# CGuerreroCordova/HydroDEM

Measured on AMD Instinct MI355X. Metric: Mcells/s sink-fill+D8 on 16384^2 float32 DEM, higher is better.
Workload: dtype f32; 1 GPU; 16384x16384 float32 synthetic DEM (SURVEY 8d 'rough': plane + 4 sinusoids + 0.5 m noise + 0.1% pits), SinkFill eps=0 to exact convergence + D8; 16384 rows per GPU, row-block partition; rows_per_gpu=16384, cols=16384, tiles=70225, visits_unchanged=25634, visits_flat=2843, certifying_rounds=0, halo_exchanges=0

## Files before the change

### hydrodem_amd/csrc/hdem_stencil.hip

```cpp
#include "hdem_internal.h"

namespace {

constexpr int TW = 256;
constexpr int TH = 32;
template <typename T> struct tile_rows { static constexpr int value = sizeof(T) == 8 ? TH / 2 : TH; };
constexpr int LS = TW + 8;
constexpr int NT = 256;

__device__ __forceinline__ int reflect(int i, int n)
{
    while (i < 0 || i >= n) {
        if (i < 0) i = -i - 1;
        if (i >= n) i = 2 * n - 1 - i;
    }
    return i;
}

template <typename T, bool REFLECT>
__device__ __forceinline__ void stage_tile(const T *__restrict__ src, int H, int W,
                                           int y0, int x0, T *t)
{
    constexpr int THT = tile_rows<T>::value;
    constexpr int V = 16 / sizeof(T);
    constexpr int CPR = TW / V;
    typedef T vec_t __attribute__((ext_vector_type(V)));
    typedef T vecu_t __attribute__((ext_vector_type(V), aligned(sizeof(T))));
    const int tid = threadIdx.x;
    constexpr int CHUNKS = ((THT + 2) * CPR + NT - 1) / NT;
    vec_t v[CHUNKS];
#pragma unroll
    for (int j = 0; j < CHUNKS; ++j) {
        const int i = tid + j * NT;
        const int r = i / CPR, c = (i % CPR) * V;
        int gy = y0 - 1 + r;
        const int gx = x0 + c;
        const bool row_ok = gy >= 0 && gy < H;
        if (REFLECT) gy = reflect(gy, H);
        if (i >= (THT + 2) * CPR) {
            v[j] = vec_t(T(0));
        } else if ((row_ok || REFLECT) && gx + V <= W) {
            v[j] = *reinterpret_cast<const vecu_t *>(src + (size_t)gy * W + gx);
        } else {
            for (int k = 0; k < V; ++k) {
                int xx = gx + k;
                T e = T(0);
                if (REFLECT) e = src[(size_t)gy * W + reflect(xx, W)];
                else if (row_ok && xx < W) e = src[(size_t)gy * W + xx];
                v[j][k] = e;
            }
        }
    }
#pragma unroll
    for (int j = 0; j < CHUNKS; ++j) {
        const int i = tid + j * NT;
        if (i < (THT + 2) * CPR)
            *reinterpret_cast<vec_t *>(t + (i / CPR) * LS + 4 + (i % CPR) * V) = v[j];
    }
    for (int i = tid; i < (THT + 2) * 2; i += NT) {
        int r = i >> 1, side = i & 1;
        int gy = y0 - 1 + r, gx = side ? x0 + TW : x0 - 1;
        T e = T(0);
        if (REFLECT) e = src[(size_t)reflect(gy, H) * W + reflect(gx, W)];
        else if (gy >= 0 && gy < H && gx >= 0 && gx < W) e = src[(size_t)gy * W + gx];
        t[r * LS + (side ? 4 + TW : 3)] = e;
    }
}

template <typename T>
__device__ __forceinline__ void read_row6(const T *t, int r, int cg, T (&o)[6])
{
    const T *p = t + r * LS + 4 + 4 * cg;
    o[0] = p[-1];
    o[1] = p[0]; o[2] = p[1]; o[3] = p[2]; o[4] = p[3];
    o[5] = p[4];
}

__device__ __forceinline__ unsigned d8_code(float nw, float n, float ne, float w,
                                            float c, float e, float sw, float s,
                                            float se)
{
    const float dg = 0.70710678f;
    float best = 0.0f;
    unsigned code = 0;
    float d;
    d = (c - nw) * dg; if (d > best) { best = d; code = 32; }
    d = (c - n);       if (d > best) { best = d; code = 64; }
    d = (c - ne) * dg; if (d > best) { best = d; code = 128; }
    d = (c - w);       if (d > best) { best = d; code = 16; }
    d = (c - e);       if (d > best) { best = d; code = 1; }
    d = (c - sw) * dg; if (d > best) { best = d; code = 8; }
    d = (c - s);       if (d > best) { best = d; code = 4; }
    d = (c - se) * dg; if (d > best) { best = d; code = 2; }
    return code;
}

__global__ __launch_bounds__(NT) void d8_kernel(const float *__restrict__ z, int H,
                                               int W, uint8_t *__restrict__ out,
                                               int tiles_x, int vec_store)
{
    __shared__ __attribute__((aligned(16))) float t[(TH + 2) * LS];
    const int bx = blockIdx.x % tiles_x, by = blockIdx.x / tiles_x;
    const int x0 = bx * TW, y0 = by * TH;
    stage_tile<float, false>(z, H, W, y0, x0, t);
    __syncthreads();

    const int cg = threadIdx.x & 63, rg = threadIdx.x >> 6;
    const int x = x0 + 4 * cg;
    if (x >= W) return;
    float a[6], b[6], c[6];
    read_row6(t, rg * 8 + 0, cg, a);
    read_row6(t, rg * 8 + 1, cg, b);
#pragma unroll
    for (int rr = 0; rr < 8; ++rr) {
        const int y = y0 + rg * 8 + rr;
        read_row6(t, rg * 8 + rr + 2, cg, c);
        if (y < H) {
            unsigned code[4];
#pragma unroll
            for (int k = 0; k < 4; ++k) {
                unsigned cd = d8_code(a[k], a[k + 1], a[k + 2], b[k], b[k + 1],
                                      b[k + 2], c[k], c[k + 1], c[k + 2]);
                int xx = x + k;
                bool interior = y > 0 && y < H - 1 && xx > 0 && xx < W - 1;
                code[k] = interior ? cd : 0u;
            }
            uint8_t *o = out + (size_t)y * W + x;
            if (vec_store && x + 4 <= W) {
                *reinterpret_cast<uint32_t *>(o) =
                    code[0] | (code[1] << 8) | (code[2] << 16) | (code[3] << 24);
            } else {
#pragma unroll
                for (int k = 0; k < 4; ++k)
                    if (x + k < W) o[k] = (uint8_t)code[k];
            }
        }
#pragma unroll
        for (int k = 0; k < 6; ++k) { a[k] = b[k]; b[k] = c[k]; }
    }
}

template <bool HAS_EPS>
__global__ __launch_bounds__(NT) void certify_d8_kernel(const float *__restrict__ z,
                                                       const float *__restrict__ w, int H, int W,
                                                       float eps, uint8_t *__restrict__ out,
                                                       int tiles_x, int vec_store, int *flag)
{
    __shared__ __attribute__((aligned(16))) float t[(TH + 2) * LS];
    const int bx = blockIdx.x % tiles_x, by = blockIdx.x / tiles_x;
    const int x0 = bx * TW, y0 = by * TH;
    stage_tile<float, false>(w, H, W, y0, x0, t);
    __syncthreads();

    const int cg = threadIdx.x & 63, rg = threadIdx.x >> 6;
    const int x = x0 + 4 * cg;
    if (x >= W) return;
    float zc[8][4];
#pragma unroll
    for (int rr = 0; rr < 8; ++rr) {
        const int y = min(y0 + rg * 8 + rr, H - 1);
        if (x + 4 <= W) {
            const hdem_f4 m = hdem_ld4u(z + (size_t)y * W + x);
            zc[rr][0] = m[0]; zc[rr][1] = m[1]; zc[rr][2] = m[2]; zc[rr][3] = m[3];
        } else {
#pragma unroll
            for (int k = 0; k < 4; ++k) zc[rr][k] = z[(size_t)y * W + min(x + k, W - 1)];
        }
    }
    bool lower = false;
    float a[6], b[6], c[6];
    read_row6(t, rg * 8 + 0, cg, a);
    read_row6(t, rg * 8 + 1, cg, b);
#pragma unroll
    for (int rr = 0; rr < 8; ++rr) {
        const int y = y0 + rg * 8 + rr;
        read_row6(t, rg * 8 + rr + 2, cg, c);
        if (y < H) {
            unsigned code[4];
#pragma unroll
            for (int k = 0; k < 4; ++k) {
                const int xx = x + k;
                const bool interior = y > 0 && y < H - 1 && xx > 0 && xx < W - 1;
                float m = fminf(fminf(fminf(a[k], a[k + 1]), fminf(a[k + 2], b[k])),
                                fminf(fminf(b[k + 1], b[k + 2]), fminf(c[k], fminf(c[k + 1], c[k + 2]))));
                m = fminf(m, HDEM_INF);
                if (HAS_EPS) m += eps;
                const float wc = fminf(b[k + 1], HDEM_INF), zz = fminf(zc[rr][k], HDEM_INF);
                lower |= interior && __builtin_amdgcn_fmed3f(zz, wc, m) != wc;
                const unsigned cd = d8_code(a[k], a[k + 1], a[k + 2], b[k], b[k + 1], b[k + 2], c[k],
                                            c[k + 1], c[k + 2]);
                code[k] = interior ? cd : 0u;
            }
            if (out) {
                uint8_t *o = out + (size_t)y * W + x;
                if (vec_store && x + 4 <= W) {
                    *reinterpret_cast<uint32_t *>(o) =
                        code[0] | (code[1] << 8) | (code[2] << 16) | (code[3] << 24);
                } else {
#pragma unroll
                    for (int k = 0; k < 4; ++k)
                        if (x + k < W) o[k] = (uint8_t)code[k];
                }
            }
        }
#pragma unroll
        for (int k = 0; k < 6; ++k) { a[k] = b[k]; b[k] = c[k]; }
    }
    if (lower) *flag = 1;
}

template <typename T>
__device__ __forceinline__ T mean9(const T (&a)[6], const T (&b)[6], const T (&c)[6],
                                   int k, int do_round)
{
    double acc = 0.0;
    acc += (double)a[k]; acc += (double)a[k + 1]; acc += (double)a[k + 2];
    acc += (double)b[k]; acc += (double)b[k + 1]; acc += (double)b[k + 2];
    acc += (double)c[k]; acc += (double)c[k + 1]; acc += (double)c[k + 2];
    T s = (T)acc;
    T m = s / T(9);
    if (do_round) m = sizeof(T) == 4 ? (T)rintf((float)m) : (T)rint((double)m);
    return m;
}

template <typename T>
__global__ __launch_bounds__(NT) void boxmean3_kernel(const T *__restrict__ x, int H,
                                                     int W, T *__restrict__ out,
                                                     int tiles_x, int do_round)
{
    constexpr int THT = tile_rows<T>::value;
    constexpr int RPW = THT / 4;
    __shared__ __attribute__((aligned(16))) T t[(THT + 2) * LS];
    const int bx = blockIdx.x % tiles_x, by = blockIdx.x / tiles_x;
    const int x0 = bx * TW, y0 = by * THT;
    stage_tile<T, true>(x, H, W, y0, x0, t);
    __syncthreads();

    const int cg = threadIdx.x & 63, rg = threadIdx.x >> 6;
    const int xc = x0 + 4 * cg;
    if (xc >= W) return;
    T a[6], b[6], c[6];
    read_row6(t, rg * RPW + 0, cg, a);
    read_row6(t, rg * RPW + 1, cg, b);
#pragma unroll
    for (int rr = 0; rr < RPW; ++rr) {
        const int y = y0 + rg * RPW + rr;
        read_row6(t, rg * RPW + rr + 2, cg, c);
        if (y < H) {
            T m[4];
#pragma unroll
            for (int k = 0; k < 4; ++k) m[k] = mean9<T>(a, b, c, k, do_round);
            T *o = out + (size_t)y * W + xc;
            if (xc + 4 <= W) {
                if (sizeof(T) == 4) {
                    hdem_f4 v = {(float)m[0], (float)m[1], (float)m[2], (float)m[3]};
                    hdem_st4u(reinterpret_cast<float *>(o), v);
                } else {
                    o[0] = m[0]; o[1] = m[1]; o[2] = m[2]; o[3] = m[3];
                }
            } else {
#pragma unroll
                for (int k = 0; k < 4; ++k)
                    if (xc + k < W) o[k] = m[k];
            }
        }
#pragma unroll
        for (int k = 0; k < 6; ++k) { a[k] = b[k]; b[k] = c[k]; }
    }
}

template <typename T>
__global__ __launch_bounds__(NT) void convolve_kernel(const T *__restrict__ x, int H,
                                                     int W, const double *__restrict__ wt,
                                                     int kh, int kw, T *__restrict__ out)
{
    size_t i = (size_t)blockIdx.x * NT + threadIdx.x;
    if (i >= (size_t)H * W) return;
    int y = (int)(i / W), xx = (int)(i % W);
    int py = kh / 2, px = kw / 2;
    double acc = 0.0;
    for (int j = 0; j < kh; ++j) {
        int gy = reflect(y + j - py, H);
        for (int k = 0; k < kw; ++k) {
            double w = wt[(kh - 1 - j) * kw + (kw - 1 - k)];
            if (w != 0.0)
                acc += (double)x[(size_t)gy * W + reflect(xx + k - px, W)] * w;
        }
    }
    const T s = (T)acc;
    out[i] = s / (T)(kh * kw);
}

template <typename T>
__global__ __launch_bounds__(NT) void around_kernel(const T *x, int64_t n, T *out)
{
    int64_t i = (int64_t)blockIdx.x * NT + threadIdx.x;
    if (i < n) out[i] = sizeof(T) == 4 ? (T)rintf((float)x[i]) : (T)rint((double)x[i]);
}

inline int tiles_of(int H, int W, int th, int *tx)
{
    *tx = (W + TW - 1) / TW;
    return *tx * ((H + th - 1) / th);
}

}

int hdem_certify_d8_launch(hdem_ctx *ctx, const float *z, const float *w, int H, int W, float eps,
                           uint8_t *d8, int *flag)
{
    int tx, nt = tiles_of(H, W, TH, &tx);
    const int vec = d8 && (W % 4 == 0) && ((uintptr_t)d8 % 4 == 0);
    if (eps != 0.0f)
        hipLaunchKernelGGL(certify_d8_kernel<true>, dim3(nt), dim3(NT), 0, ctx->stream, z, w, H, W,
                           eps, d8, tx, vec, flag);
    else
        hipLaunchKernelGGL(certify_d8_kernel<false>, dim3(nt), dim3(NT), 0, ctx->stream, z, w, H, W,
                           eps, d8, tx, vec, flag);
    HDEM_HIP_CHECK(hipGetLastError());
    return HDEM_OK;
}

extern "C" int hdem_d8_f32_dev(hdem_ctx *ctx, const float *z, int H, int W, uint8_t *out)
{
    if (int rc = hdem_check_call(ctx, z, out, H, W)) return rc;
    HDEM_HIP_CHECK(hipSetDevice(ctx->device));
    int tx, nt = tiles_of(H, W, TH, &tx);
    int vec = (W % 4 == 0) && ((uintptr_t)out % 4 == 0);
    {
        hdem_scoped_timer tm(ctx, HDEM_K_D8, (int64_t)H * W);
        hipLaunchKernelGGL(d8_kernel, dim3(nt), dim3(NT), 0, ctx->stream, z, H, W, out,
                           tx, vec);
    }
    HDEM_HIP_CHECK(hipGetLastError());
    return HDEM_OK;
}

extern "C" int hdem_d8_f32(hdem_ctx *ctx, const float *z, int H, int W, uint8_t *out)
{
    if (int rc = hdem_check_call(ctx, z, out, H, W)) return rc;
    HDEM_HIP_CHECK(hipSetDevice(ctx->device));
    size_t n = (size_t)H * W;
    hdem_dbuf dz, dout;
    if (int rc = dz.upload(ctx, z, n * sizeof(float))) return rc;
    if (int rc = dout.alloc(ctx, n)) return rc;
    if (int rc = hdem_d8_f32_dev(ctx, dz.as<const float>(), H, W, dout.as<uint8_t>())) return rc;
    return dout.download(out, n);
}

template <typename T>
static int boxmean_dev(hdem_ctx *ctx, const T *x, int H, int W, int do_round, T *out)
{
    if (int rc = hdem_check_call(ctx, x, out, H, W)) return rc;
    HDEM_REQUIRE((const void *)x != (const void *)out, HDEM_ERR_BAD_ARG,
                 "box mean cannot run in place");
    HDEM_HIP_CHECK(hipSetDevice(ctx->device));
    int tx, nt = tiles_of(H, W, tile_rows<T>::value, &tx);
    {
        hdem_scoped_timer tm(ctx, HDEM_K_BOXMEAN, (int64_t)H * W);
        hipLaunchKernelGGL(boxmean3_kernel<T>, dim3(nt), dim3(NT), 0, ctx->stream, x, H, W,
                           out, tx, do_round);
    }
    HDEM_HIP_CHECK(hipGetLastError());
    return HDEM_OK;
}

template <typename T>
static int boxmean_host(hdem_ctx *ctx, const T *x, int H, int W, int do_round, T *out)
{
    if (int rc = hdem_check_call(ctx, x, out, H, W)) return rc;
    HDEM_HIP_CHECK(hipSetDevice(ctx->device));
    size_t bytes = (size_t)H * W * sizeof(T);
    hdem_dbuf dx, dout;
    if (int rc = dx.upload(ctx, x, bytes)) return rc;
    if (int rc = dout.alloc(ctx, bytes)) return rc;
    if (int rc = boxmean_dev<T>(ctx, dx.as<const T>(), H, W, do_round, dout.as<T>())) return rc;
    return dout.download(out, bytes);
}

extern "C" int hdem_boxmean3_f32_dev(hdem_ctx *c, const float *x, int H, int W, int r, float *o)
{ return boxmean_dev<float>(c, x, H, W, r, o); }
extern "C" int hdem_boxmean3_f64_dev(hdem_ctx *c, const double *x, int H, int W, int r, double *o)
{ return boxmean_dev<double>(c, x, H, W, r, o); }
extern "C" int hdem_boxmean3_f32(hdem_ctx *c, const float *x, int H, int W, int r, float *o)
{ return boxmean_host<float>(c, x, H, W, r, o); }
extern "C" int hdem_boxmean3_f64(hdem_ctx *c, const double *x, int H, int W, int r, double *o)
{ return boxmean_host<double>(c, x, H, W, r, o); }

template <typename T>
static int convolve_host(hdem_ctx *ctx, const T *x, int H, int W, const double *weights, int kh,
                         int kw, T *out)
{
    if (int rc = hdem_check_call(ctx, x, out, H, W)) return rc;
    HDEM_REQUIRE(weights, HDEM_ERR_BAD_ARG, "weights is null");
    HDEM_REQUIRE(kh > 0 && kw > 0 && kh <= 15 && kw <= 15, HDEM_ERR_BAD_ARG,
                 "weights shape %d x %d not supported (1..15 per axis)", kh, kw);
    HDEM_REQUIRE(kh % 2 == 1 && kw % 2 == 1, HDEM_ERR_WINDOW_EVEN,
                 "weights shape %d x %d must be odd on both axes", kh, kw);
    HDEM_HIP_CHECK(hipSetDevice(ctx->device));
    size_t n = (size_t)H * W, bytes = n * sizeof(T);
    hdem_dbuf dx, dout, dw;
    if (int rc = dx.upload(ctx, x, bytes)) return rc;
    if (int rc = dw.upload(ctx, weights, sizeof(double) * kh * kw)) return rc;
    if (int rc = dout.alloc(ctx, bytes)) return rc;
    {
        hdem_scoped_timer tm(ctx, HDEM_K_CONVOLVE, (int64_t)n);
        hipLaunchKernelGGL(convolve_kernel<T>, dim3((unsigned)((n + NT - 1) / NT)), dim3(NT), 0,
                           ctx->stream, dx.as<const T>(), H, W, dw.as<const double>(), kh, kw,
                           dout.as<T>());
    }
    HDEM_HIP_CHECK(hipGetLastError());
    return dout.download(out, bytes);
}

extern "C" int hdem_convolve_f32(hdem_ctx *ctx, const float *x, int H, int W,
                                 const double *weights, int kh, int kw, float *out)
{ return convolve_host<float>(ctx, x, H, W, weights, kh, kw, out); }
extern "C" int hdem_convolve_f64(hdem_ctx *ctx, const double *x, int H, int W,
                                 const double *weights, int kh, int kw, double *out)
{ return convolve_host<double>(ctx, x, H, W, weights, kh, kw, out); }

template <typename T>
static int around_host(hdem_ctx *ctx, const T *x, int64_t n, T *out)
{
    HDEM_REQUIRE(ctx && x && out, HDEM_ERR_BAD_ARG, "null argument");
    HDEM_REQUIRE(n > 0, HDEM_ERR_BAD_ARG, "n must be positive");
    HDEM_HIP_CHECK(hipSetDevice(ctx->device));
    const size_t bytes = (size_t)n * sizeof(T);
    hdem_dbuf dx;
    if (int rc = dx.upload(ctx, x, bytes)) return rc;
    hipLaunchKernelGGL(around_kernel<T>, dim3((unsigned)((n + NT - 1) / NT)), dim3(NT), 0,
                       ctx->stream, dx.as<const T>(), n, dx.as<T>());
    HDEM_HIP_CHECK(hipGetLastError());
    return dx.download(out, bytes);
}

extern "C" int hdem_around_f32(hdem_ctx *c, const float *x, int64_t n, float *o)
{ return around_host<float>(c, x, n, o); }
extern "C" int hdem_around_f64(hdem_ctx *c, const double *x, int64_t n, double *o)
{ return around_host<double>(c, x, n, o); }
```

Baseline: 63880 Mcells/s.

## Share neighbor slope differences across rows and batch D8 stores

Restructures the D8 and certify-D8 kernels so that vertical and diagonal differences between adjacent rows are computed once and reused by the rows above and below. Direction selection becomes a max reduction followed by equality-based code selection. For eps=0 the certify check is reduced to a cheaper comparison built from the drop mask. Codes for all 8 rows are buffered in registers and stored at the end, with sched_barriers to control instruction scheduling. This trims ALU work and branching per cell, at the cost of more registers and a tie-breaking rule that must match the original strict-greater ordering.

After: 63790 Mcells/s. About the same (-0.1%).

```diff
diff --git a/hydrodem_amd/csrc/hdem_stencil.hip b/hydrodem_amd/csrc/hdem_stencil.hip
--- a/hydrodem_amd/csrc/hdem_stencil.hip
+++ b/hydrodem_amd/csrc/hdem_stencil.hip
@@ -76,23 +76,88 @@
     o[5] = p[4];
 }
 
-__device__ __forceinline__ unsigned d8_code(float nw, float n, float ne, float w,
-                                            float c, float e, float sw, float s,
-                                            float se)
+struct d8_link {
+    float v[4];
+    float dr[5];
+    float dl[5];
+};
+
+__device__ __forceinline__ void d8_link_rows(const float (&u)[6], const float (&l)[6],
+                                             d8_link &s)
 {
     const float dg = 0.70710678f;
-    float best = 0.0f;
-    unsigned code = 0;
-    float d;
-    d = (c - nw) * dg; if (d > best) { best = d; code = 32; }
-    d = (c - n);       if (d > best) { best = d; code = 64; }
-    d = (c - ne) * dg; if (d > best) { best = d; code = 128; }
-    d = (c - w);       if (d > best) { best = d; code = 16; }
-    d = (c - e);       if (d > best) { best = d; code = 1; }
-    d = (c - sw) * dg; if (d > best) { best = d; code = 8; }
-    d = (c - s);       if (d > best) { best = d; code = 4; }
-    d = (c - se) * dg; if (d > best) { best = d; code = 2; }
-    return code;
+#pragma unroll
+    for (int k = 0; k < 4; ++k) s.v[k] = u[k + 1] - l[k + 1];
+#pragma unroll
+    for (int j = 0; j < 5; ++j) {
+        s.dr[j] = (u[j] - l[j + 1]) * dg;
+        s.dl[j] = (u[j + 1] - l[j]) * dg;
+    }
+}
+
+__device__ __forceinline__ void d8_row4(const float (&b)[6], const d8_link &n,
+                                        const d8_link &s, unsigned (&code)[4],
+                                        bool (&drop)[4])
+{
+    float h[5];
+#pragma unroll
+    for (int j = 0; j < 5; ++j) h[j] = b[j] - b[j + 1];
+#pragma unroll
+    for (int k = 0; k < 4; ++k) {
+        const float d0 = -n.dr[k], d1 = -n.v[k], d2 = -n.dl[k + 1], d3 = -h[k];
+        const float d4 = h[k + 1], d5 = s.dl[k], d6 = s.v[k], d7 = s.dr[k + 1];
+        float m = __builtin_fmaxf(__builtin_fmaxf(d0, d1), d2);
+        m = __builtin_fmaxf(__builtin_fmaxf(m, d3), d4);
+        m = __builtin_fmaxf(__builtin_fmaxf(m, d5), d6);
+        m = __builtin_fmaxf(m, d7);
+        unsigned cd = d7 == m ? 2u : 0u;
+        cd = d6 == m ? 4u : cd;
+        cd = d5 == m ? 8u : cd;
+        cd = d4 == m ? 1u : cd;
+        cd = d3 == m ? 16u : cd;
+        cd = d2 == m ? 128u : cd;
+        cd = d1 == m ? 64u : cd;
+        cd = d0 == m ? 32u : cd;
+        code[k] = cd;
+        drop[k] = m > 0.0f;
+    }
+}
+
+__device__ __forceinline__ unsigned d8_column_mask(int x, int W)
+{
+    unsigned m = 0;
+#pragma unroll
+    for (int k = 0; k < 4; ++k)
+        m |= (x + k > 0 && x + k < W - 1) ? 0xffu << (8 * k) : 0u;
+    return m;
+}
+
+__device__ __forceinline__ unsigned d8_word(const unsigned (&code)[4], const bool (&drop)[4],
+                                            unsigned cmask, int y, int H)
+{
+    const unsigned word = (drop[0] ? code[0] : 0u) | (drop[1] ? code[1] << 8 : 0u) |
+                          (drop[2] ? code[2] << 16 : 0u) | (drop[3] ? code[3] << 24 : 0u);
+    unsigned r = (y > 0 && y < H - 1) ? word & cmask : 0u;
+    asm volatile("" : "+v"(r));
+    return r;
+}
+
+__device__ __forceinline__ void d8_store_rows(uint8_t *__restrict__ out, int H, int W, int y,
+                                              int x, int vec_store, const unsigned (&word)[8])
+{
+    if (vec_store && x + 4 <= W) {
+#pragma unroll
+        for (int rr = 0; rr < 8; ++rr)
+            if (y + rr < H)
+                *reinterpret_cast<uint32_t *>(out + (size_t)(y + rr) * W + x) = word[rr];
+    } else {
+#pragma unroll
+        for (int rr = 0; rr < 8; ++rr)
+#pragma unroll
+            for (int k = 0; k < 4; ++k)
+                if (y + rr < H && x + k < W)
+                    out[(size_t)(y + rr) * W + x + k] = (uint8_t)(word[rr] >> (8 * k));
+    }
 }
 
 __global__ __launch_bounds__(NT) void d8_kernel(const float *__restrict__ z, int H,
@@ -108,36 +173,29 @@
     const int cg = threadIdx.x & 63, rg = threadIdx.x >> 6;
     const int x = x0 + 4 * cg;
     if (x >= W) return;
+    unsigned cmask = 0;
+#pragma unroll
+    for (int k = 0; k < 4; ++k) cmask |= (x + k > 0 && x + k < W - 1) ? 0xffu << (8 * k) : 0u;
+    unsigned word[8];
     float a[6], b[6], c[6];
+    d8_link ln, ls;
     read_row6(t, rg * 8 + 0, cg, a);
     read_row6(t, rg * 8 + 1, cg, b);
+    d8_link_rows(a, b, ln);
 #pragma unroll
     for (int rr = 0; rr < 8; ++rr) {
-        const int y = y0 + rg * 8 + rr;
+        unsigned code[4];
+        bool drop[4];
         read_row6(t, rg * 8 + rr + 2, cg, c);
-        if (y < H) {
-            unsigned code[4];
-#pragma unroll
-            for (int k = 0; k < 4; ++k) {
-                unsigned cd = d8_code(a[k], a[k + 1], a[k + 2], b[k], b[k + 1],
-                                      b[k + 2], c[k], c[k + 1], c[k + 2]);
-                int xx = x + k;
-                bool interior = y > 0 && y < H - 1 && xx > 0 && xx < W - 1;
-                code[k] = interior ? cd : 0u;
-            }
-            uint8_t *o = out + (size_t)y * W + x;
-            if (vec_store && x + 4 <= W) {
-                *reinterpret_cast<uint32_t *>(o) =
-                    code[0] | (code[1] << 8) | (code[2] << 16) | (code[3] << 24);
-            } else {
-#pragma unroll
-                for (int k = 0; k < 4; ++k)
-                    if (x + k < W) o[k] = (uint8_t)code[k];
-            }
-        }
-#pragma unroll
-        for (int k = 0; k < 6; ++k) { a[k] = b[k]; b[k] = c[k]; }
-    }
+        d8_link_rows(b, c, ls);
+        d8_row4(b, ln, ls, code, drop);
+        word[rr] = d8_word(code, drop, cmask, y0 + rg * 8 + rr, H);
+        ln = ls;
+#pragma unroll
+        for (int k = 0; k < 6; ++k) b[k] = c[k];
+        __builtin_amdgcn_sched_barrier(0);
+    }
+    d8_store_rows(out, H, W, y0 + rg * 8, x, vec_store, word);
 }
 
 template <bool HAS_EPS>
@@ -167,46 +225,52 @@
             for (int k = 0; k < 4; ++k) zc[rr][k] = z[(size_t)y * W + min(x + k, W - 1)];
         }
     }
+    unsigned cmask = 0;
+    bool colin[4];
+#pragma unroll
+    for (int k = 0; k < 4; ++k) {
+        colin[k] = x + k > 0 && x + k < W - 1;
+        cmask |= colin[k] ? 0xffu << (8 * k) : 0u;
+    }
     bool lower = false;
+    unsigned word[8];
     float a[6], b[6], c[6];
+    d8_link ln, ls;
     read_row6(t, rg * 8 + 0, cg, a);
     read_row6(t, rg * 8 + 1, cg, b);
+    d8_link_rows(a, b, ln);
 #pragma unroll
     for (int rr = 0; rr < 8; ++rr) {
         const int y = y0 + rg * 8 + rr;
+        unsigned code[4];
+        bool drop[4], low[4];
         read_row6(t, rg * 8 + rr + 2, cg, c);
-        if (y < H) {
-            unsigned code[4];
-#pragma unroll
-            for (int k = 0; k < 4; ++k) {
-                const int xx = x + k;
-                const bool interior = y > 0 && y < H - 1 && xx > 0 && xx < W - 1;
+        d8_link_rows(b, c, ls);
+        d8_row4(b, ln, ls, code, drop);
+#pragma unroll
+        for (int k = 0; k < 4; ++k) {
+            const float wk = b[k + 1], zk = zc[rr][k];
+            if (HAS_EPS) {
                 float m = fminf(fminf(fminf(a[k], a[k + 1]), fminf(a[k + 2], b[k])),
                                 fminf(fminf(b[k + 1], b[k + 2]), fminf(c[k], fminf(c[k + 1], c[k + 2]))));
                 m = fminf(m, HDEM_INF);
-                if (HAS_EPS) m += eps;
-                const float wc = fminf(b[k + 1], HDEM_INF), zz = fminf(zc[rr][k], HDEM_INF);
-                lower |= interior && __builtin_amdgcn_fmed3f(zz, wc, m) != wc;
-                const unsigned cd = d8_code(a[k], a[k + 1], a[k + 2], b[k], b[k + 1], b[k + 2], c[k],
-                                            c[k + 1], c[k + 2]);
-                code[k] = interior ? cd : 0u;
-            }
-            if (out) {
-                uint8_t *o = out + (size_t)y * W + x;
-                if (vec_store && x + 4 <= W) {
-                    *reinterpret_cast<uint32_t *>(o) =
-                        code[0] | (code[1] << 8) | (code[2] << 16) | (code[3] << 24);
-                } else {
-#pragma unroll
-                    for (int k = 0; k < 4; ++k)
-                        if (x + k < W) o[k] = (uint8_t)code[k];
-                }
+                m += eps;
+                const float wc = fminf(wk, HDEM_INF), zz = fminf(zk, HDEM_INF);
+                low[k] = __builtin_amdgcn_fmed3f(zz, wc, m) != wc;
+            } else {
+                low[k] = (drop[k] & (zk < wk)) | (!(wk >= zk) & (zk == zk));
             }
         }
+        lower |= (y > 0 && y < H - 1) &
+                 ((low[0] & colin[0]) | (low[1] & colin[1]) | (low[2] & colin[2]) | (low[3] & colin[3]));
+        word[rr] = d8_word(code, drop, cmask, y, H);
+        ln = ls;
 #pragma unroll
         for (int k = 0; k < 6; ++k) { a[k] = b[k]; b[k] = c[k]; }
+        __builtin_amdgcn_sched_barrier(0);
     }
     if (lower) *flag = 1;
+    if (out) d8_store_rows(out, H, W, y0 + rg * 8, x, vec_store, word);
 }
 
 template <typename T>
```
